# zwpku/colvars-finder

Measured on AMD Instinct MI355X. Metric: MD frames/sec through EigenFunctionTask train step, higher is better.
Workload: dtype f32; 1 GPU; BASELINE config 3: alanine-dipeptide-shaped EigenFunctionTask, generator mode, k=3, 22 atoms, align+position features d_r=66, nets [66,20,20,20,1], diag_coeff, Adam; frames_per_gpu=100000, batch_per_gpu=20000, global_batch=20000, parallelism=dp1 (frames sharded; all-reduce of batch sums + flat gradient)

## Files before the change

### colvars-finder_amd/csrc/ef16_back.hip

```cpp
#include "ef16_common.hpp"

namespace {

struct Back16Args {
  int k;
  int64_t B;
  int64_t n_tiles;
  int64_t T;
  const float* w_lag;
};

template <int H, int NH, bool MULTI, bool GEN>
__global__ __launch_bounds__(256, 4) void ef16_back_kernel(Back16Args args, cvf_mlp_desc mlp, const float* __restrict__ theta,
                                                            const float* __restrict__ packed, const float* __restrict__ w,
                                                            const float* __restrict__ feat, const float* __restrict__ y_tiled,
                                                            const float* __restrict__ q_tiled, const double* __restrict__ coef,
                                                            float* __restrict__ slab, int32_t* __restrict__ step,
                                                            const float* __restrict__ saved) {
  constexpr int RT = Hid<H>::RT, NG = Hid<H>::NG;
  constexpr int RTO = (H + 15) / 16;
  constexpr int CTH = (H + 1 + 15) / 16;
  constexpr int NT = 256, WPB = 4;
  constexpr int kRows = 2 * H + 2 * (H + 1) + 16;
  __shared__ __attribute__((aligned(16))) float IMG[kRows * kPitch];
  __shared__ float PART[4 * (H + 1)];
  extern __shared__ float GI[];
  float* SA1 = IMG;
  float* SA2 = SA1 + H * kPitch;
  float* SB1 = SA2 + H * kPitch;
  float* SB2 = SB1 + (H + 1) * kPitch;
  const int tid = threadIdx.x, lane = tid & 63;
  const int wave = __builtin_amdgcn_readfirstlane(tid >> 6);
  const int col = lane & 15, q = lane >> 4, row16 = col, r0 = 4 * q;
  const int fo = 16 * wave + col;
  const int rowf = 4 * col + q;
  const int net = blockIdx.y, k = args.k, D = mlp.dims[0];
  const int CT1 = (D + 1 + 15) / 16;
  const int c0 = 16 * (CT1 - 1), nfeat = D - c0, ncol = nfeat + 1;
  const bool strip = ncol <= 4;
  const int CTM = strip ? CT1 - 1 : CT1;
  const int gbase = mlp.w_off[net][0];
  const int gspan = mlp.b_off[net][NH] + 1 - gbase;
  float* out = slab + (int64_t)blockIdx.x * mlp.n_params + gbase;

  {
    static_assert((kRows * kPitch) % 4 == 0, "IMG is zeroed in 16-byte pieces");
    float4* img4 = reinterpret_cast<float4*>(IMG);
    for (int i = tid; i < kRows * kPitch / 4; i += NT) img4[i] = float4{0.0f, 0.0f, 0.0f, 0.0f};
  }
  if (MULTI)
    for (int i = tid; i < gspan; i += NT) GI[i] = 0.0f;
  lds_barrier();
  if (tid < 64) SB1[H * kPitch + tid] = 1.0f;

  const PackLayout L = pack_layout(H, NH, D);
  const URows pk = urows(packed + (int64_t)net * L.per_net, L.per_net, lane);
  float wl[RT][4];
  load_hid_const_u<H>(urows(theta + mlp.w_off[net][NH], H, q), wl);
  const double gS1n = coef[net], gEtn = coef[k + k * k + net];
  const double gS1ln = GEN ? 0.0 : coef[2 * k + k * k + net], gS2ln = GEN ? 0.0 : coef[3 * k + k * k + net];
  const float one[1] = {1.0f};

  const __amdgpu_buffer_rsrc_t out_rs = __builtin_amdgcn_make_buffer_rsrc(out, 0, gspan * 4, 0x00020000);
  auto emit_tile = [&](int l, int n_out, int n_in, int rt, int ct, const f32x4& acc) {
    const int wo = mlp.w_off[net][l] - gbase, bo = mlp.b_off[net][l] - gbase;
    const int i = 16 * ct + row16;
    int ob = 16 * rt + r0;
    asm volatile("" : "+v"(ob));
#pragma unroll
    for (int r = 0; r < 4; ++r) {
      const int o = ob + r;
      const bool isw = o < n_out && i < n_in, isb = o < n_out && i == n_in;
      const int idx = isw ? wo + o * n_in + i : bo + (o < n_out ? o : 0);
      const float av = acc[r];
      if (MULTI) {
        if (isw || isb) GI[idx] += av;
      } else {
        __builtin_amdgcn_raw_buffer_store_b32(__builtin_bit_cast(int, av), out_rs, (isw || isb) ? idx * 4 : 0x7ffffff0, 0, 0);
      }
    }
  };
  auto outer2 = [&](const float* A1, const float* B1, const float* A2, const float* B2, int rt, int ct) {
    f32x4 acc = {0.0f, 0.0f, 0.0f, 0.0f};
    acc = outer_half(A1, B1, rt, ct, lane, acc);
    if constexpr (GEN) acc = outer_half(A2, B2, rt, ct, lane, acc);
    return acc;
  };

  auto emit_entry = [&](bool live, int idx, float v) {
    if (MULTI) {
      if (live) GI[idx] += v;
    } else {
      __builtin_amdgcn_raw_buffer_store_b32(__builtin_bit_cast(int, v), out_rs, live ? idx * 4 : 0x7ffffff0, 0, 0);
    }
  };
  auto emit_last = [&]() {
    if (wave == WPB - 1) {
      int i = lane;
      asm volatile("" : "+v"(i));
      const bool live = i <= H;
      const float v = strip_total(PART + (live ? i : H), H + 1);
      emit_entry(live, i < H ? mlp.w_off[net][NH] - gbase + i : mlp.b_off[net][NH] - gbase, v);
    }
  };
  auto emit_strip = [&]() {
    if (strip && 64 * wave < 4 * H) {
      int e = tid;
      asm volatile("" : "+v"(e));
      const int o = e >> 2, c = e & 3;
      const bool live = o < H && c < ncol;
      const float v = strip_total(SB1 + (o < H ? e : 0), 4 * H);
      emit_entry(live, c < nfeat ? mlp.w_off[net][0] - gbase + o * D + c0 + c : mlp.b_off[net][0] - gbase + o, v);
    }
  };

  for (int64_t tile = blockIdx.x; tile < args.n_tiles; tile += gridDim.x) {
    CVF_STAMP(8);
    const bool lagged = !GEN && tile >= args.T;
    const int64_t t0 = lagged ? tile - args.T : tile;
    const int64_t frame = t0 * CVF_TILE + fo;
    const bool valid = frame < args.B;
    const float wraw = w[valid ? frame : args.B - 1];
    float yb[CVF_MAX_NETS];
#pragma unroll
    for (int j = 0; j < CVF_MAX_NETS; ++j) yb[j] = y_tiled[(t0 * k + (j < k ? j : k - 1)) * CVF_TILE + fo];
    float ylag = 0.0f, wlraw = 0.0f;
    if constexpr (!GEN) {
      ylag = y_tiled[((args.T + t0) * k + net) * CVF_TILE + fo];
      wlraw = args.w_lag[valid ? frame : args.B - 1];
    }
    const URows sv = urows(saved + (tile * k + net) * (int64_t)(kHand<NH>() * NG * 256) + wave * 64, kHand<NH>() * NG * 256 - wave * 64, lane);
    Vec<H, 1> h[NH], e[NH > 1 ? NH - 1 : 1], t[NH];
#pragma unroll
    for (int l = 0; l < NH; ++l) {
#pragma unroll
      for (int rt = 0; rt < RT; ++rt) h[l].v[rt][0] = f32x4{0.0f, 0.0f, 0.0f, 0.0f};
#pragma unroll
      for (int g = 0; g < NG; ++g) h[l].v[g >> 2][0][g & 3] = sv.ld((l * NG + g) * 256);
    }
    if constexpr (GEN) {
#pragma unroll
      for (int l = 0; l + 1 < NH; ++l) {
#pragma unroll
        for (int rt = 0; rt < RT; ++rt) e[l].v[rt][0] = f32x4{0.0f, 0.0f, 0.0f, 0.0f};
#pragma unroll
        for (int g = 0; g < NG; ++g) e[l].v[g >> 2][0][g & 3] = sv.ld(((NH + l) * NG + g) * 256);
      }
#pragma unroll
      for (int rt = 0; rt < RT; ++rt) t[0].v[rt][0] = f32x4{0.0f, 0.0f, 0.0f, 0.0f};
#pragma unroll
      for (int g = 0; g < NG; ++g) t[0].v[g >> 2][0][g & 3] = sv.ld(((2 * NH - 1) * NG + g) * 256);
    }
    HFrag<H> ffr[NH > 1 ? NH - 1 : 1];
    if constexpr (GEN) {
#pragma unroll
      for (int l = 1; l < NH; ++l) load_hfrag_u<H>(ffr[l - 1], pk, L.fh(l));
    }
    const float* f_tile = feat + tile * (int64_t)D * CVF_TILE;
    const float* q_tile = GEN ? q_tiled + (tile * k + net) * (int64_t)D * CVF_TILE : nullptr;
    const float wb = valid ? wraw : 0.0f;
    float alpha, gamma = 0.0f;
    float ynet = 0.0f;
#pragma unroll
    for (int j = 0; j < CVF_MAX_NETS; ++j)
      if (j == net) ynet = yb[j];
    if (GEN || !lagged) {
      double a = gS1n;
#pragma unroll
      for (int j = 0; j < CVF_MAX_NETS; ++j)
        if (j < k) a += (j == net ? 2.0 : 1.0) * coef[k + net * k + j] * (double)yb[j];
      alpha = (float)((double)wb * a);
      if constexpr (GEN) gamma = (float)(2.0 * (double)wb * gEtn);
      else alpha = (float)((double)wb * a - 2.0 * (double)wb * gEtn * ((double)ylag - (double)ynet));
    } else {
      const double wlg = valid ? (double)wlraw : 0.0;
      alpha = (float)(wlg * (gS1ln + 2.0 * gS2ln * (double)ylag) + 2.0 * (double)wb * gEtn * ((double)ylag - (double)ynet));
    }
    CVF_STAMP(9);
    if constexpr (GEN) {
#pragma unroll
      for (int rt = 0; rt < RT; ++rt)
#pragma unroll
        for (int r = 0; r < 4; ++r) t[0].v[rt][0][r] *= gamma;
#pragma unroll
      for (int l = 1; l < NH; ++l) {
        Vec<H, 1> td;
        tangent_of<H, 1>(td, h[l - 1], t[l - 1]);
        init_bias<H, 1>(t[l], nullptr, q);
        hidden_mul<H, 1>(t[l], ffr[l - 1], td);
      }
    }
    CVF_STAMP(11);
    {
      const float pick = strip_rows<H>([&](int rt, int r) {
        const float hv = h[NH - 1].v[rt][0][r];
        if constexpr (GEN) return fmaf(alpha, hv, (1.0f - hv * hv) * t[NH - 1].v[rt][0][r]);
        else return alpha * hv;
      }, col);
      const float sa = row_sumf16(alpha);
      if (col < NG && rowf < H) PART[wave * (H + 1) + rowf] = pick;
      if (lane == 0) PART[wave * (H + 1) + H] = sa;
    }
    CVF_STAMP(12);
    Vec<H, 1> hbar;
#pragma unroll
    for (int rt = 0; rt < RT; ++rt)
#pragma unroll
      for (int r = 0; r < 4; ++r) hbar.v[rt][0][r] = alpha * wl[rt][r];
    HFrag<H> tfl;
    float4 bA[4], bB[4];
    float xs[3] = {0.0f, 0.0f, 0.0f}, qs[3] = {0.0f, 0.0f, 0.0f};
    auto request = [&](float4 (&dst)[4], const float* src_tile, int ct) {
      const int i = 16 * ct + row16;
      const float4* p = reinterpret_cast<const float4*>(src_tile + (int64_t)(i < D ? i : D - 1) * CVF_TILE + 4 * q);
#pragma unroll
      for (int j = 0; j < 4; ++j) dst[j] = p[4 * j];
    };
    auto request_step = [&](int l) {
      if (l > 0) {
        load_hfrag_u<H>(tfl, pk, L.th(l));
      } else {
        if (strip) {
#pragma unroll
          for (int c = 0; c < 3; ++c)
            if (c < nfeat) {
              xs[c] = f_tile[(int64_t)(c0 + c) * CVF_TILE + fo];
              if constexpr (GEN) qs[c] = q_tile[(int64_t)(c0 + c) * CVF_TILE + fo];
            }
        }
        request(bA, f_tile, wave);
        if constexpr (GEN) request(bB, q_tile, wave);
      }
    };
    request_step(NH - 1);
#pragma unroll
    for (int l = NH - 1; l >= 0; --l) {
      CVF_STAMP(13 + (NH - 1 - l));
      Vec<H, 1> zbar, dl;
#pragma unroll
      for (int rt = 0; rt < RT; ++rt)
#pragma unroll
        for (int r = 0; r < 4; ++r) {
          const float hv = h[l].v[rt][0][r];
          const float om = 1.0f - hv * hv;
          if constexpr (GEN) {
            const float ev = (l == NH - 1) ? wl[rt][r] : e[l < NH - 1 ? l : 0].v[rt][0][r];
            const float hb = fmaf(-2.0f * hv * t[l].v[rt][0][r], ev, hbar.v[rt][0][r]);
            dl.v[rt][0][r] = ev * om;
            zbar.v[rt][0][r] = om * hb;
          } else {
            zbar.v[rt][0][r] = om * hbar.v[rt][0][r];
          }
        }
      store_image<H, 1, false>(SA1, zbar, one, lane, fo);
      if constexpr (GEN) {
        const float sc[1] = {l == 0 ? gamma : 1.0f};
        store_image<H, 1, true>(SA2, dl, sc, lane, fo);
      }
      if (l > 0) {
        store_image<H, 1, false>(SB1, h[l - 1], one, lane, fo);
        if constexpr (GEN) {
          Vec<H, 1> td;
          tangent_of<H, 1>(td, h[l - 1], t[l - 1]);
          store_image<H, 1, false>(SB2, td, one, lane, fo);
        }
        __syncthreads();
        init_bias<H, 1>(hbar, nullptr, q);
        hidden_mul<H, 1>(hbar, tfl, zbar);
        request_step(l - 1);
        for (int pr = wave; pr < RTO * CTH; pr += WPB) {
          const int rt = pr / CTH, ct = pr - rt * CTH;
          emit_tile(l, H, H, rt, ct, outer2(SA1, SB1, SA2, SB2, rt, ct));
        }
        if (l == NH - 1) emit_last();
        __syncthreads();
      } else {
        if (strip) {
#pragma unroll
          for (int c = 0; c < 4; ++c) {
            if (c < ncol) {
              const float xv = c == nfeat ? 1.0f : xs[c < 3 ? c : 2];
              const float qv = c == nfeat ? 0.0f : gamma * qs[c < 3 ? c : 2];
              const float pick = strip_rows<H>([&](int rt, int r) {
                if constexpr (GEN) return fmaf(zbar.v[rt][0][r], xv, dl.v[rt][0][r] * qv);
                else return zbar.v[rt][0][r] * xv;
              }, col);
              if (col < NG && rowf < H) SB1[(wave * H + rowf) * 4 + c] = pick;
            }
          }
        }
        __syncthreads();
        auto half0 = [&](f32x4 (&acc)[RTO], const float* SA, const float4 (&b)[4], int ct, int rt0, int rstep, bool ones) {
          const int i = 16 * ct + row16;
          const float pad = (ones && i == D) ? 1.0f : 0.0f;
#pragma unroll
          for (int rt = 0; rt < RTO; ++rt) {
            if (rt >= rt0 && (rt - rt0) % rstep == 0) {
              const float4* a1 = reinterpret_cast<const float4*>(SA + (16 * rt + row16) * kPitch + 4 * q);
              float4 av[4];
#pragma unroll
              for (int j = 0; j < 4; ++j) av[j] = a1[4 * j];
#pragma unroll
              for (int j = 0; j < 4; ++j) {
                acc[rt] = mfma4(av[j].x, i < D ? b[j].x : pad, acc[rt]);
                acc[rt] = mfma4(av[j].y, i < D ? b[j].y : pad, acc[rt]);
                acc[rt] = mfma4(av[j].z, i < D ? b[j].z : pad, acc[rt]);
                acc[rt] = mfma4(av[j].w, i < D ? b[j].w : pad, acc[rt]);
              }
            }
          }
        };
        const int extra = (CTM - WPB) * RTO;
        f32x4 acc[RTO];
#pragma unroll
        for (int rt = 0; rt < RTO; ++rt) acc[rt] = f32x4{0.0f, 0.0f, 0.0f, 0.0f};
        if (wave < CTM) {
          half0(acc, SA1, bA, wave, 0, 1, true);
          if (wave < extra) request(bA, f_tile, WPB + wave / RTO);
          if constexpr (GEN) half0(acc, SA2, bB, wave, 0, 1, false);
#pragma unroll
          for (int rt = 0; rt < RTO; ++rt) emit_tile(0, H, D, rt, wave, acc[rt]);
        }
        for (int pr = wave; pr < extra; pr += WPB) {
          const int ct = WPB + pr / RTO, rt = pr % RTO;
          if (pr != wave || wave >= CTM) request(bA, f_tile, ct);
          if constexpr (GEN) request(bB, q_tile, ct);
#pragma unroll
          for (int r_ = 0; r_ < RTO; ++r_) acc[r_] = f32x4{0.0f, 0.0f, 0.0f, 0.0f};
          half0(acc, SA1, bA, ct, rt, RTO, true);
          if constexpr (GEN) half0(acc, SA2, bB, ct, rt, RTO, false);
#pragma unroll
          for (int r_ = 0; r_ < RTO; ++r_)
            if (r_ == rt) emit_tile(0, H, D, r_, ct, acc[r_]);
        }
        emit_strip();
        if (NH == 1) emit_last();
        __syncthreads();
      }
    }
  }
  CVF_STAMP(17);
  if (MULTI) {
    __syncthreads();
    for (int i = tid; i < gspan; i += NT) out[i] = GI[i];
  }
  if (step != nullptr && blockIdx.x == 0 && blockIdx.y == 0 && tid == 0) *step += 1;
  CVF_STAMP(18);
}

}

extern "C" int64_t cvf_ef16_backward_slab_rows(int64_t n_tiles) { return n_tiles < 1024 ? n_tiles : 1024; }

static int ef16_backward_impl(const cvf_ef_cfg* cfg, const cvf_mlp_desc* mlp, const float* theta, const float* packed,
                              int64_t B, const float* w, const float* w_lag, const float* feat_tiled, const float* y_tiled,
                              const float* q_tiled, const double* coef, float* slab, int32_t* step_count, const float* saved,
                              void* stream) {
  const bool transfer = cfg != nullptr && cfg->lag_idx > 0;
  CVF_REQUIRE(cfg && mlp && theta && packed && w && feat_tiled && y_tiled && (transfer ? w_lag != nullptr : q_tiled != nullptr) && coef &&
              slab && saved && B > 0, "cvf_ef16_backward: bad argument");
  CVF_REQUIRE(cfg->k == mlp->n_nets, "cvf_ef16_backward: cfg.k must equal the number of nets");
  int H, NH;
  CVF_REQUIRE(ef16_shape(mlp, &H, &NH), "cvf_ef16_backward: unsupported net shape");
  CVF_REQUIRE(mlp->dims[0] <= 8 * 16 - 1, "cvf_ef16_backward: first layer wider than the column-tile schedule covers");
  const int span = mlp->b_off[0][NH] + 1 - mlp->w_off[0][0];
  int covered = 0;
  for (int n = 0; n < mlp->n_nets; ++n) {
    CVF_REQUIRE(mlp->b_off[n][NH] + 1 - mlp->w_off[n][0] == span, "cvf_ef16_backward: nets are not laid out contiguously");
    for (int l = 0; l <= NH; ++l)
      CVF_REQUIRE(mlp->w_off[n][l] >= mlp->w_off[n][0] && mlp->b_off[n][l] < mlp->w_off[n][0] + span,
                  "cvf_ef16_backward: nets are not laid out contiguously");
    covered += span;
  }
  CVF_REQUIRE(covered == mlp->n_params, "cvf_ef16_backward: flat buffer holds parameters outside the nets");
  Back16Args a;
  a.k = cfg->k;
  a.B = B;
  a.T = cvf_ntiles(B);
  a.n_tiles = transfer ? 2 * a.T : a.T;
  a.w_lag = w_lag;
  const int64_t G = cvf_ef16_backward_slab_rows(a.n_tiles);
  const bool launched = ef16_dispatch(H, NH, [&](auto h_, auto nh_) {
    constexpr int kH = decltype(h_)::value, kNH = decltype(nh_)::value;
    auto go = [&](auto kernel, size_t lds) {
      hipLaunchKernelGGL(kernel, dim3((unsigned)G, cfg->k), dim3(256), lds, (hipStream_t)stream, a, *mlp, theta, packed, w, feat_tiled,
                         y_tiled, q_tiled, coef, slab, step_count, saved);
    };
    const size_t gi = (size_t)span * sizeof(float);
    if (transfer) {
      if (a.n_tiles > G) go(ef16_back_kernel<kH, kNH, true, false>, gi);
      else go(ef16_back_kernel<kH, kNH, false, false>, 0);
    } else {
      if (a.n_tiles > G) go(ef16_back_kernel<kH, kNH, true, true>, gi);
      else go(ef16_back_kernel<kH, kNH, false, true>, 0);
    }
  });
  CVF_REQUIRE(launched, "cvf_ef16_backward: no kernel instance for hidden width %d x %d layers", H, NH);
  return cvf_check_launch("ef16_back_kernel");
}

extern "C" int cvf_ef16_backward(const cvf_ef_cfg* cfg, const cvf_mlp_desc* mlp, const float* theta, const float* packed,
                                 int64_t B, const float* w, const float* feat_tiled, const float* y_tiled, const float* q_tiled,
                                 const double* coef, float* slab, int32_t* step_count, const float* saved, void* stream) {
  CVF_REQUIRE(cfg && cfg->lag_idx == 0, "cvf_ef16_backward: generator mode (transfer-operator mode: cvf_ef16_backward_transfer)");
  return ef16_backward_impl(cfg, mlp, theta, packed, B, w, nullptr, feat_tiled, y_tiled, q_tiled, coef, slab, step_count, saved, stream);
}


extern "C" int cvf_ef16_backward_transfer(const cvf_ef_cfg* cfg, const cvf_mlp_desc* mlp, const float* theta, const float* packed,
                                          int64_t B, const float* w, const float* w_lag, const float* feat_tiled,
                                          const float* y_tiled, const double* coef, float* slab, int32_t* step_count,
                                          const float* saved, void* stream) {
  CVF_REQUIRE(cfg && cfg->lag_idx > 0, "cvf_ef16_backward_transfer: transfer-operator mode (cfg.lag_idx > 0)");
  return ef16_backward_impl(cfg, mlp, theta, packed, B, w, w_lag, feat_tiled, y_tiled, nullptr, coef, slab, step_count, saved, stream);
}
```

### colvars-finder_amd/csrc/ef16_common.hpp

```cpp
#pragma once
#include "cvf_metric.hpp"
#include "ef_frag.hpp"
#include <stdlib.h>
#include <type_traits>


namespace {

constexpr int kU = 16;
constexpr int kImgP = 76;
constexpr int kAuxP = 21;
constexpr int kMaxRows16 = 16384;
template <int NH>
__host__ __device__ constexpr int kHand() { return 2 * NH; }

__device__ __forceinline__ float quad_sumf16(float v) {
  v += dpp_movf<0xB1, 0xf>(v);
  v += dpp_movf<0x4E, 0xf>(v);
  return v;
}
__device__ __forceinline__ double quad_sumd16(double v) {
  v += dpp_movd<0xB1, 0xf>(v);
  v += dpp_movd<0x4E, 0xf>(v);
  return v;
}

__device__ __forceinline__ float row_sumf16(float v) {
  v = quad_sumf16(v);
  v += dpp_movf<0x141, 0xf>(v);
  v += dpp_movf<0x140, 0xf>(v);
  return v;
}
template <int H, class F>
__device__ __forceinline__ float strip_rows(F&& val, int col) {
  float pick = 0.0f;
#pragma unroll
  for (int j = 0; j < Hid<H>::NG; ++j) {
    const float s = row_sumf16(val(j >> 2, j & 3));
    pick = col == j ? s : pick;
  }
  return pick;
}
__device__ __forceinline__ float strip_total(const float* P, int stride) {
  return ((P[0] + P[stride]) + P[2 * stride]) + P[3 * stride];
}

struct Front16Lds {
  int ref, a, aux, w, rs, y, e, feat, g, total;
};
__host__ __device__ inline Front16Lds front16_lds(int nc, int nal, int k) {
  Front16Lds L;
  const int stride = x_tile_stride(nc);
  L.ref = kU * stride;
  L.a = L.ref + 3 * nal;
  L.aux = (L.a + nc + 3) & ~3;
  L.w = L.aux + ((kU * kAuxP + 3) & ~3);
  L.rs = L.w + kU;
  L.y = L.rs + 4;
  L.e = L.y + k * kU;
  L.feat = L.e + k * kU;
  L.g = L.feat + kU * kImgP;
  L.total = L.g + k * kU * kImgP;
  return L;
}

bool ef16_shape(const cvf_mlp_desc* m, int* H, int* NH) {
  if (m->n_layers < 2 || m->n_layers > 4 || m->dims[m->n_layers] != 1) return false;
  *H = m->dims[1];
  *NH = m->n_layers - 1;
  for (int l = 1; l < m->n_layers; ++l)
    if (m->dims[l] != *H) return false;
  for (int l = 0; l < m->n_layers; ++l)
    if (m->act[l] != (l + 1 < m->n_layers ? 1 : 0)) return false;
  return true;
}

template <class F>
bool ef16_dispatch(int H, int NH, F&& f) {
#define EF_CASE(H_, NH_)                                                        \
  if (H == H_ && NH == NH_) {                                                   \
    f(std::integral_constant<int, H_>{}, std::integral_constant<int, NH_>{});   \
    return true;                                                                \
  }
#ifdef CVF_DEV_SHAPES
  EF_CASE(20, 3)
#else
  EF_CASE(8, 1) EF_CASE(8, 2) EF_CASE(8, 3)
  EF_CASE(12, 1) EF_CASE(12, 2) EF_CASE(12, 3)
  EF_CASE(16, 1) EF_CASE(16, 2) EF_CASE(16, 3)
  EF_CASE(20, 1) EF_CASE(20, 2) EF_CASE(20, 3)
  EF_CASE(24, 2) EF_CASE(24, 3)
  EF_CASE(32, 2) EF_CASE(32, 3)
#endif
#undef EF_CASE
  return false;
}

}
```

### colvars-finder_amd/csrc/ef_frag.hpp

```cpp
#pragma once
#include "cvf_common.hpp"
#include "cvf_pack.hpp"

namespace {

typedef float f32x4 __attribute__((ext_vector_type(4)));


constexpr int kPitch = 68;

__device__ __forceinline__ f32x4 mfma4(float a, float b, f32x4 c) {
  return __builtin_amdgcn_mfma_f32_16x16x4f32(a, b, c, 0, 0, 0);
}

template <int H>
struct Hid {
  static constexpr int NG = (H + 3) / 4;
  static constexpr int RT = (NG + 3) / 4;
};

template <int H, int FT>
struct Vec {
  f32x4 v[Hid<H>::RT][FT];
};

template <int H>
__host__ __device__ constexpr int saved_per_vec() { return Hid<H>::NG * 2 * 64 * 2; }
template <int H>
__device__ __forceinline__ void save_vec(float* __restrict__ base, const Vec<H, 4>& X, int lane) {
#pragma unroll
  for (int g = 0; g < Hid<H>::NG; ++g)
#pragma unroll
    for (int w = 0; w < 2; ++w)
      reinterpret_cast<float2*>(base + (g * 2 + w) * 128)[lane] = float2{X.v[g >> 2][2 * w][g & 3], X.v[g >> 2][2 * w + 1][g & 3]};
}
template <int H>
__device__ __forceinline__ void save_vec_half(float* __restrict__ base, const Vec<H, 2>& X, int w, int lane) {
#pragma unroll
  for (int g = 0; g < Hid<H>::NG; ++g)
    reinterpret_cast<float2*>(base + (g * 2 + w) * 128)[lane] = float2{X.v[g >> 2][0][g & 3], X.v[g >> 2][1][g & 3]};
}
template <int H>
__device__ __forceinline__ void load_vec(const float* __restrict__ base, Vec<H, 2>& X, int w, int lane) {
#pragma unroll
  for (int rt = 0; rt < Hid<H>::RT; ++rt)
#pragma unroll
    for (int ft = 0; ft < 2; ++ft) X.v[rt][ft] = f32x4{0.0f, 0.0f, 0.0f, 0.0f};
#pragma unroll
  for (int g = 0; g < Hid<H>::NG; ++g) {
    const float2 t = reinterpret_cast<const float2*>(base + (g * 2 + w) * 128)[lane];
    X.v[g >> 2][0][g & 3] = t.x;
    X.v[g >> 2][1][g & 3] = t.y;
  }
}

template <int H, int FT>
__device__ __forceinline__ void init_bias(Vec<H, FT>& X, const float* __restrict__ b, int q) {
#pragma unroll
  for (int rt = 0; rt < Hid<H>::RT; ++rt) {
    f32x4 bv;
#pragma unroll
    for (int r = 0; r < 4; ++r) {
      const int f = hid_feature(rt, r, q);
      bv[r] = 0.0f;
      if (b != nullptr) {
        const float x = b[f < H ? f : H - 1];
        bv[r] = f < H ? x : 0.0f;
      }
    }
#pragma unroll
    for (int ft = 0; ft < FT; ++ft) X.v[rt][ft] = bv;
  }
}

template <int FT>
__device__ __forceinline__ void load_frames(const float* __restrict__ p, float (&b)[FT]) {
  if constexpr (FT == 4) {
    const float4 v = *reinterpret_cast<const float4*>(p);
    b[0] = v.x; b[1] = v.y; b[2] = v.z; b[3] = v.w;
  } else if constexpr (FT == 2) {
    const float2 v = *reinterpret_cast<const float2*>(p);
    b[0] = v.x; b[1] = v.y;
  } else {
    b[0] = p[0];
  }
}
template <int FT>
__device__ __forceinline__ void store_frames(float* __restrict__ p, const float (&b)[FT]) {
  if constexpr (FT == 4) *reinterpret_cast<float4*>(p) = make_float4(b[0], b[1], b[2], b[3]);
  else if constexpr (FT == 2) *reinterpret_cast<float2*>(p) = make_float2(b[0], b[1]);
  else p[0] = b[0];
}


template <int H>
struct HFrag {
  float a[Hid<H>::NG][Hid<H>::RT];
};
template <int H>
__device__ __forceinline__ void load_hfrag(HFrag<H>& f, const float* __restrict__ pk, int lane) {
#pragma unroll
  for (int s = 0; s < Hid<H>::NG; ++s)
#pragma unroll
    for (int rt = 0; rt < Hid<H>::RT; ++rt) f.a[s][rt] = pk[(unsigned)((s * Hid<H>::RT + rt) * 64) + (unsigned)lane];
}
template <int H, int FT>
__device__ __forceinline__ void hidden_mul(Vec<H, FT>& Y, const HFrag<H>& f, const Vec<H, FT>& X) {
#pragma unroll
  for (int s = 0; s < Hid<H>::NG; ++s)
#pragma unroll
    for (int ft = 0; ft < FT; ++ft)
#pragma unroll
      for (int rt = 0; rt < Hid<H>::RT; ++rt) Y.v[rt][ft] = mfma4(f.a[s][rt], X.v[s >> 2][ft][s & 3], Y.v[rt][ft]);
}
template <int H, int FT>
__device__ __forceinline__ void hidden_apply(Vec<H, FT>& Y, const float* __restrict__ pk, const Vec<H, FT>& X, int lane) {
  HFrag<H> f;
  load_hfrag<H>(f, pk, lane);
  hidden_mul<H, FT>(Y, f, X);
}

template <int H, int FT, int CH>
struct L0Chunk {
  float a[CH][Hid<H>::RT];
  float b[CH][FT];
};
template <int H, int FT, int CH>
__device__ __forceinline__ void load_l0chunk(L0Chunk<H, FT, CH>& c, const float* __restrict__ pk0, int D, int S,
                                             const float* __restrict__ in_lane, int s0, int lane) {
  constexpr int RT = Hid<H>::RT;
  const int q = lane >> 4;
#pragma unroll
  for (int i = 0; i < CH; ++i) {
    const int s = s0 + i;
    const bool live = s < S;
    const int se = live ? s : S - 1;
    const int kf = 4 * se + q;
#pragma unroll
    for (int rt = 0; rt < RT; ++rt) {
#ifdef CVF_EXP_NOW
      const float v = 0.01f * (float)(se + rt);
#else
      const float v = pk0[(se * RT + rt) * 64 + lane];
#endif
      c.a[i][rt] = live ? v : 0.0f;
    }
#ifdef CVF_EXP_NOFEAT
#pragma unroll
    for (int ft = 0; ft < FT; ++ft) c.b[i][ft] = 0.5f + 0.01f * (float)kf;
#else
    load_frames<FT>(in_lane + (int64_t)(kf < D ? kf : 0) * CVF_TILE, c.b[i]);
#endif
  }
}
template <int H, int FT, int CH>
__device__ __forceinline__ void mul_l0chunk(Vec<H, FT>& X, const L0Chunk<H, FT, CH>& c) {
#pragma unroll
  for (int i = 0; i < CH; ++i)
#pragma unroll
    for (int ft = 0; ft < FT; ++ft)
#pragma unroll
      for (int rt = 0; rt < Hid<H>::RT; ++rt) X.v[rt][ft] = mfma4(c.a[i][rt], c.b[i][ft], X.v[rt][ft]);
}
template <int H, int FT, int CH = 6>
__device__ __forceinline__ void layer0_apply(Vec<H, FT>& X, const float* __restrict__ pk0, int D,
                                             const float* __restrict__ in_lane, int lane) {
  const int S = (D + 3) >> 2;
  L0Chunk<H, FT, CH> c0, c1;
  load_l0chunk<H, FT, CH>(c0, pk0, D, S, in_lane, 0, lane);
  for (int s0 = 0; s0 < S; s0 += 2 * CH) {
    load_l0chunk<H, FT, CH>(c1, pk0, D, S, in_lane, s0 + CH, lane);
    mul_l0chunk<H, FT, CH>(X, c0);
    load_l0chunk<H, FT, CH>(c0, pk0, D, S, in_lane, s0 + 2 * CH, lane);
    mul_l0chunk<H, FT, CH>(X, c1);
  }
}

template <int H, int FT, int CH, int NB>
__device__ __forceinline__ void layer0_apply_deep(Vec<H, FT>& X, const float* __restrict__ pk0, int D,
                                                  const float* __restrict__ in_lane, int lane) {
  const int S = (D + 3) >> 2;
  L0Chunk<H, FT, CH> c[NB];
#pragma unroll
  for (int b = 0; b < NB; ++b) load_l0chunk<H, FT, CH>(c[b], pk0, D, S, in_lane, b * CH, lane);
  for (int s0 = 0; s0 < S; s0 += NB * CH) {
#pragma unroll
    for (int b = 0; b < NB; ++b) {
      mul_l0chunk<H, FT, CH>(X, c[b]);
      load_l0chunk<H, FT, CH>(c[b], pk0, D, S, in_lane, s0 + (NB + b) * CH, lane);
    }
  }
}
constexpr int kWideD = 128;

template <int H, int FT, int CH>
__device__ __forceinline__ void layer0_apply_from(Vec<H, FT>& X, const float* __restrict__ pk0, int D,
                                                  const float* __restrict__ in_lane, int lane, L0Chunk<H, FT, CH>& c0) {
  const int S = (D + 3) >> 2;
  L0Chunk<H, FT, CH> c1;
  for (int s0 = 0; s0 < S; s0 += 2 * CH) {
    load_l0chunk<H, FT, CH>(c1, pk0, D, S, in_lane, s0 + CH, lane);
    mul_l0chunk<H, FT, CH>(X, c0);
    load_l0chunk<H, FT, CH>(c0, pk0, D, S, in_lane, s0 + 2 * CH, lane);
    mul_l0chunk<H, FT, CH>(X, c1);
  }
}

template <int H>
struct HConst {
  float c[Hid<H>::RT][4];
};
template <int H>
__device__ __forceinline__ void load_hconst(HConst<H>& o, const float* __restrict__ v, int q) {
#pragma unroll
  for (int rt = 0; rt < Hid<H>::RT; ++rt)
#pragma unroll
    for (int r = 0; r < 4; ++r) {
      const int f = hid_feature(rt, r, q);
      const float x = v[f < H ? f : H - 1];
      o.c[rt][r] = f < H ? x : 0.0f;
    }
}
template <int H, int FT>
__device__ __forceinline__ void set_const(Vec<H, FT>& X, const HConst<H>& b) {
#pragma unroll
  for (int rt = 0; rt < Hid<H>::RT; ++rt)
#pragma unroll
    for (int ft = 0; ft < FT; ++ft)
#pragma unroll
      for (int r = 0; r < 4; ++r) X.v[rt][ft][r] = b.c[rt][r];
}

__device__ __attribute__((noinline)) float ef_act_slow(int act, float z) { return cvf_act(act, z); }
__device__ __attribute__((noinline)) float ef_act_d1_slow(int act, float h) { return cvf_act_d1(act, h); }
__device__ __attribute__((noinline)) float ef_act_d2_slow(int act, float h) { return cvf_act_d2(act, h); }

template <int H, int FT>
__device__ __forceinline__ void tanh_inplace(Vec<H, FT>& X, int act = CVF_ACT_TANH) {
  if (act == CVF_ACT_TANH) {
#pragma unroll
    for (int rt = 0; rt < Hid<H>::RT; ++rt)
#pragma unroll
      for (int ft = 0; ft < FT; ++ft)
#pragma unroll
        for (int r = 0; r < 4; ++r)
          if (4 * rt + r < Hid<H>::NG) X.v[rt][ft][r] = cvf_tanh(X.v[rt][ft][r]);
  } else {
#pragma unroll
    for (int rt = 0; rt < Hid<H>::RT; ++rt)
#pragma unroll
      for (int ft = 0; ft < FT; ++ft)
#pragma unroll
        for (int r = 0; r < 4; ++r)
          if (4 * rt + r < Hid<H>::NG) X.v[rt][ft][r] = ef_act_slow(act, X.v[rt][ft][r]);
  }
}
__device__ __forceinline__ float act_d1(int act, float h) {
  if (act == CVF_ACT_TANH) return 1.0f - h * h;
  return ef_act_d1_slow(act, h);
}

template <int H>
__device__ __forceinline__ void load_hid_const(const float* __restrict__ v, int q, float (&c)[Hid<H>::RT][4]) {
#pragma unroll
  for (int rt = 0; rt < Hid<H>::RT; ++rt)
#pragma unroll
    for (int r = 0; r < 4; ++r) {
      const int f = hid_feature(rt, r, q);
      const float x = v[f < H ? f : H - 1];
      c[rt][r] = f < H ? x : 0.0f;
    }
}

template <int H, int NH, int FT, bool LEAN = false>
__device__ __forceinline__ void chain_forward(const cvf_mlp_desc& mlp, const float* __restrict__ theta,
                                              const float* __restrict__ pk, const PackLayout& L, int net,
                                              const float* __restrict__ in_lane, int lane, Vec<H, FT> (&h)[NH]) {
  const int q = lane >> 4;
  if constexpr (LEAN) {
    init_bias<H, FT>(h[0], theta + mlp.b_off[net][0], q);
    layer0_apply<H, FT, 3>(h[0], pk + L.f0(), mlp.dims[0], in_lane, lane);
    tanh_inplace<H, FT>(h[0], mlp.act[0]);
#pragma unroll
    for (int l = 1; l < NH; ++l) {
      init_bias<H, FT>(h[l], theta + mlp.b_off[net][l], q);
      hidden_apply<H, FT>(h[l], pk + L.fh(l), h[l - 1], lane);
      tanh_inplace<H, FT>(h[l], mlp.act[0]);
    }
    return;
  }
  HConst<H> bias[NH];
#pragma unroll
  for (int l = 0; l < NH; ++l) load_hconst<H>(bias[l], theta + mlp.b_off[net][l], q);
  HFrag<H> hf[NH > 1 ? NH - 1 : 1];
#pragma unroll
  for (int l = 1; l < NH; ++l) load_hfrag<H>(hf[l - 1], pk + L.fh(l), lane);
  CVF_STAMP(1);
  set_const<H, FT>(h[0], bias[0]);
  if (mlp.dims[0] > kWideD) layer0_apply_deep<H, FT, 6, 3>(h[0], pk + L.f0(), mlp.dims[0], in_lane, lane);
  else layer0_apply<H, FT>(h[0], pk + L.f0(), mlp.dims[0], in_lane, lane);
  CVF_STAMP(2);
  tanh_inplace<H, FT>(h[0], mlp.act[0]);
  CVF_STAMP(3);
#pragma unroll
  for (int l = 1; l < NH; ++l) {
    set_const<H, FT>(h[l], bias[l]);
    hidden_mul<H, FT>(h[l], hf[l - 1], h[l - 1]);
    tanh_inplace<H, FT>(h[l], mlp.act[0]);
  }
}

__device__ __forceinline__ float sum_over_q(float v) {
  v += __shfl_xor(v, 16, 64);
  v += __shfl_xor(v, 32, 64);
  return v;
}

struct URows {
  __amdgpu_buffer_rsrc_t r;
  int lane4;
  __device__ __forceinline__ float ld(int float_off) const {
    return __builtin_bit_cast(float, __builtin_amdgcn_raw_buffer_load_b32(r, lane4, float_off * 4, 0));
  }
  __device__ __forceinline__ void st(int float_off, float v) const {
    __builtin_amdgcn_raw_buffer_store_b32(__builtin_bit_cast(int, v), r, lane4, float_off * 4, 0);
  }
};
__device__ __forceinline__ URows urows(const void* base, int n_floats, int lane) {
  return URows{__builtin_amdgcn_make_buffer_rsrc(const_cast<void*>(base), 0, n_floats * 4, 0x00020000), lane * 4};
}
template <int H>
__device__ __forceinline__ void load_hfrag_u(HFrag<H>& f, const URows& u, int off) {
#pragma unroll
  for (int s = 0; s < Hid<H>::NG; ++s)
#pragma unroll
    for (int rt = 0; rt < Hid<H>::RT; ++rt) f.a[s][rt] = u.ld(off + (s * Hid<H>::RT + rt) * 64);
}
template <int H>
__device__ __forceinline__ void load_hid_const_u(const URows& u, float (&c)[Hid<H>::RT][4]) {
#pragma unroll
  for (int rt = 0; rt < Hid<H>::RT; ++rt)
#pragma unroll
    for (int r = 0; r < 4; ++r) c[rt][r] = u.ld(4 * (4 * rt + r));
}

__device__ __forceinline__ f32x4 outer_half(const float* __restrict__ A, const float* __restrict__ B, int rt, int ct,
                                            int lane, f32x4 acc) {
  const int row = lane & 15, kq = lane >> 4;
  const float4* a = reinterpret_cast<const float4*>(A + (16 * rt + row) * kPitch + 4 * kq);
  const float4* b = reinterpret_cast<const float4*>(B + (16 * ct + row) * kPitch + 4 * kq);
  float4 av[4], bv[4];
#pragma unroll
  for (int j = 0; j < 4; ++j) {
    av[j] = a[4 * j];
    bv[j] = b[4 * j];
  }
#pragma unroll
  for (int j = 0; j < 4; ++j) {
    acc = mfma4(av[j].x, bv[j].x, acc);
    acc = mfma4(av[j].y, bv[j].y, acc);
    acc = mfma4(av[j].z, bv[j].z, acc);
    acc = mfma4(av[j].w, bv[j].w, acc);
  }
  return acc;
}
__device__ __forceinline__ f32x4 outer_tile(const float* __restrict__ A1, const float* __restrict__ B1,
                                            const float* __restrict__ A2, const float* __restrict__ B2, int rt, int ct,
                                            bool two, int lane) {
  f32x4 acc = {0.0f, 0.0f, 0.0f, 0.0f};
  acc = outer_half(A1, B1, rt, ct, lane, acc);
  if (two) acc = outer_half(A2, B2, rt, ct, lane, acc);
  return acc;
}

template <int H, int FT, bool SCALE>
__device__ __forceinline__ void store_image(float* S, const Vec<H, FT>& X, const float (&sc)[FT], int lane, int fo) {
  const int q = lane >> 4;
#pragma unroll
  for (int rt = 0; rt < Hid<H>::RT; ++rt)
#pragma unroll
    for (int r = 0; r < 4; ++r) {
      const int f = hid_feature(rt, r, q);
      if (4 * rt + r < Hid<H>::NG && f < H) {
        float v[FT];
#pragma unroll
        for (int ft = 0; ft < FT; ++ft) v[ft] = SCALE ? sc[ft] * X.v[rt][ft][r] : X.v[rt][ft][r];
        float* dst = S + f * kPitch + fo;
        if constexpr (FT == 4) {
          reinterpret_cast<float2*>(dst)[0] = make_float2(v[0], v[1]);
          reinterpret_cast<float2*>(dst)[1] = make_float2(v[2], v[3]);
        } else if constexpr (FT == 2) {
          *reinterpret_cast<float2*>(dst) = make_float2(v[0], v[1]);
        } else {
          dst[0] = v[0];
        }
      }
    }
}

template <int H, int FT>
__device__ __forceinline__ void tangent_of(Vec<H, FT>& td, const Vec<H, FT>& h, const Vec<H, FT>& t, int act = CVF_ACT_TANH) {
  if (act == CVF_ACT_TANH) {
#pragma unroll
    for (int rt = 0; rt < Hid<H>::RT; ++rt)
#pragma unroll
      for (int ft = 0; ft < FT; ++ft)
#pragma unroll
        for (int r = 0; r < 4; ++r) {
          const float hv = h.v[rt][ft][r];
          td.v[rt][ft][r] = (1.0f - hv * hv) * t.v[rt][ft][r];
        }
  } else {
#pragma unroll
    for (int rt = 0; rt < Hid<H>::RT; ++rt)
#pragma unroll
      for (int ft = 0; ft < FT; ++ft)
#pragma unroll
        for (int r = 0; r < 4; ++r) td.v[rt][ft][r] = ef_act_d1_slow(act, h.v[rt][ft][r]) * t.v[rt][ft][r];
  }
}

}
```

Baseline: 328.6 million frames/s.

## Compute ragged hidden-size tail of weight-gradient tiles with 4x4x1 MFMA

When the hidden width leaves a small tail (H mod 16 in 1..4, e.g. H=20), the backward kernel stops computing full 16x16 outer-product tiles for the mostly-empty second row tile. It uses 4x4x1 MFMA blocks instead, then reduces them with permlane swaps and scatters the entries straight into the gradient. Roles rotate across waves by layer parity to balance the work. This cuts wasted MFMA work on padding, at the cost of more complex indexing, extra cross-lane reductions and possible load imbalance between waves.

```diff
diff --git a/colvars-finder_amd/csrc/ef16_back.hip b/colvars-finder_amd/csrc/ef16_back.hip
--- a/colvars-finder_amd/csrc/ef16_back.hip
+++ b/colvars-finder_amd/csrc/ef16_back.hip
@@ -21,6 +21,7 @@
   constexpr int RTO = (H + 15) / 16;
   constexpr int CTH = (H + 1 + 15) / 16;
   constexpr int NT = 256, WPB = 4;
+  constexpr bool TAIL4 = RTO == 2 && H % 16 >= 1 && H % 16 <= 4;
   constexpr int kRows = 2 * H + 2 * (H + 1) + 16;
   __shared__ __attribute__((aligned(16))) float IMG[kRows * kPitch];
   __shared__ float PART[4 * (H + 1)];
@@ -268,9 +269,32 @@
         init_bias<H, 1>(hbar, nullptr, q);
         hidden_mul<H, 1>(hbar, tfl, zbar);
         request_step(l - 1);
-        for (int pr = wave; pr < RTO * CTH; pr += WPB) {
-          const int rt = pr / CTH, ct = pr - rt * CTH;
-          emit_tile(l, H, H, rt, ct, outer2(SA1, SB1, SA2, SB2, rt, ct));
+        if constexpr (TAIL4) {
+          const int role = (wave + 2 * (l & 1)) & 3;
+          if (role == 0) {
+            emit_tile(l, H, H, 0, 0, outer2(SA1, SB1, SA2, SB2, 0, 0));
+          } else {
+            const int g = col >> 2, m = lane & 3;
+            const int wo = mlp.w_off[net][l] - gbase, bo = mlp.b_off[net][l] - gbase;
+            auto job = [&](int arow, int brow, int o, int i, bool live) {
+              f32x4 acc = {0.0f, 0.0f, 0.0f, 0.0f};
+              acc = outer_half44(SA1, arow, SB1, brow, lane, acc);
+              if constexpr (GEN) acc = outer_half44(SA2, arow, SB2, brow, lane, acc);
+              const float v = rows_sum_scatter(acc);
+              asm volatile("" : "+v"(o));
+              live = live && o < H && i <= H;
+              emit_entry(live, i < H ? wo + o * H + i : bo + o, v);
+            };
+            const bool low = role == 1;
+            const int cb = role == 3 ? 20 : 16;
+            job(low ? 16 + m : 4 * g + m, low ? 4 * g + m : cb + m, low ? 16 + q : 4 * g + q, low ? 4 * g + m : cb + m, true);
+            if (low) job(16 + m, 16 + 4 * (g & 1) + m, 16 + q, 16 + 4 * (g & 1) + m, g < 2);
+          }
+        } else {
+          for (int pr = wave; pr < RTO * CTH; pr += WPB) {
+            const int rt = pr / CTH, ct = pr - rt * CTH;
+            emit_tile(l, H, H, rt, ct, outer2(SA1, SB1, SA2, SB2, rt, ct));
+          }
         }
         if (l == NH - 1) emit_last();
         __syncthreads();
@@ -314,12 +338,40 @@
         f32x4 acc[RTO];
 #pragma unroll
         for (int rt = 0; rt < RTO; ++rt) acc[rt] = f32x4{0.0f, 0.0f, 0.0f, 0.0f};
+        auto tail0 = [&](f32x4& tacc, const float* SA, const float4 (&b)[4], int ct, bool ones) {
+          const int i = 16 * ct + row16;
+          const float pad = (ones && i == D) ? 1.0f : 0.0f;
+          const float4* a1 = reinterpret_cast<const float4*>(SA + (16 + (lane & 3)) * kPitch + 4 * q);
+          float4 av[4];
+#pragma unroll
+          for (int j = 0; j < 4; ++j) av[j] = a1[4 * j];
+#pragma unroll
+          for (int j = 0; j < 4; ++j) {
+            tacc = mfma1(av[j].x, i < D ? b[j].x : pad, tacc);
+            tacc = mfma1(av[j].y, i < D ? b[j].y : pad, tacc);
+            tacc = mfma1(av[j].z, i < D ? b[j].z : pad, tacc);
+            tacc = mfma1(av[j].w, i < D ? b[j].w : pad, tacc);
+          }
+        };
         if (wave < CTM) {
-          half0(acc, SA1, bA, wave, 0, 1, true);
+          f32x4 tacc = {0.0f, 0.0f, 0.0f, 0.0f};
+          half0(acc, SA1, bA, wave, 0, TAIL4 ? RTO : 1, true);
+          if constexpr (TAIL4) tail0(tacc, SA1, bA, wave, true);
           if (wave < extra) request(bA, f_tile, WPB + wave / RTO);
-          if constexpr (GEN) half0(acc, SA2, bB, wave, 0, 1, false);
-#pragma unroll
-          for (int rt = 0; rt < RTO; ++rt) emit_tile(0, H, D, rt, wave, acc[rt]);
+          if constexpr (GEN) {
+            half0(acc, SA2, bB, wave, 0, TAIL4 ? RTO : 1, false);
+            if constexpr (TAIL4) tail0(tacc, SA2, bB, wave, false);
+          }
+#pragma unroll
+          for (int rt = 0; rt < (TAIL4 ? 1 : RTO); ++rt) emit_tile(0, H, D, rt, wave, acc[rt]);
+          if constexpr (TAIL4) {
+            const float v = rows_sum_scatter(tacc);
+            int o = 16 + q;
+            asm volatile("" : "+v"(o));
+            const int i = 16 * wave + row16;
+            const bool isw = o < H && i < D, isb = o < H && i == D;
+            emit_entry(isw || isb, isw ? mlp.w_off[net][0] - gbase + o * D + i : mlp.b_off[net][0] - gbase + (o < H ? o : 0), v);
+          }
         }
         for (int pr = wave; pr < extra; pr += WPB) {
           const int ct = WPB + pr / RTO, rt = pr % RTO;
diff --git a/colvars-finder_amd/csrc/ef16_common.hpp b/colvars-finder_amd/csrc/ef16_common.hpp
--- a/colvars-finder_amd/csrc/ef16_common.hpp
+++ b/colvars-finder_amd/csrc/ef16_common.hpp
@@ -43,6 +43,17 @@
 }
 __device__ __forceinline__ float strip_total(const float* P, int stride) {
   return ((P[0] + P[stride]) + P[2 * stride]) + P[3 * stride];
+}
+
+__device__ __forceinline__ float rows_sum_scatter(const f32x4& x) {
+  auto swap_add = [](auto swapped) {
+    const unsigned a = swapped[0], b = swapped[1];
+    return __builtin_bit_cast(float, a) + __builtin_bit_cast(float, b);
+  };
+  const float x0 = x[0], x1 = x[1], x2 = x[2], x3 = x[3];
+  const float s02 = swap_add(__builtin_amdgcn_permlane32_swap(__builtin_bit_cast(unsigned, x0), __builtin_bit_cast(unsigned, x2), false, false));
+  const float s13 = swap_add(__builtin_amdgcn_permlane32_swap(__builtin_bit_cast(unsigned, x1), __builtin_bit_cast(unsigned, x3), false, false));
+  return swap_add(__builtin_amdgcn_permlane16_swap(__builtin_bit_cast(unsigned, s02), __builtin_bit_cast(unsigned, s13), false, false));
 }
 
 struct Front16Lds {
diff --git a/colvars-finder_amd/csrc/ef_frag.hpp b/colvars-finder_amd/csrc/ef_frag.hpp
--- a/colvars-finder_amd/csrc/ef_frag.hpp
+++ b/colvars-finder_amd/csrc/ef_frag.hpp
@@ -11,6 +11,9 @@
 
 __device__ __forceinline__ f32x4 mfma4(float a, float b, f32x4 c) {
   return __builtin_amdgcn_mfma_f32_16x16x4f32(a, b, c, 0, 0, 0);
+}
+__device__ __forceinline__ f32x4 mfma1(float a, float b, f32x4 c) {
+  return __builtin_amdgcn_mfma_f32_4x4x1f32(a, b, c, 0, 0, 0);
 }
 
 template <int H>
@@ -364,6 +367,26 @@
   }
   return acc;
 }
+__device__ __forceinline__ f32x4 outer_half44(const float* __restrict__ A, int arow, const float* __restrict__ B, int brow,
+                                              int lane, f32x4 acc) {
+  const int kq = lane >> 4;
+  const float4* a = reinterpret_cast<const float4*>(A + arow * kPitch + 4 * kq);
+  const float4* b = reinterpret_cast<const float4*>(B + brow * kPitch + 4 * kq);
+  float4 av[4], bv[4];
+#pragma unroll
+  for (int j = 0; j < 4; ++j) {
+    av[j] = a[4 * j];
+    bv[j] = b[4 * j];
+  }
+#pragma unroll
+  for (int j = 0; j < 4; ++j) {
+    acc = mfma1(av[j].x, bv[j].x, acc);
+    acc = mfma1(av[j].y, bv[j].y, acc);
+    acc = mfma1(av[j].z, bv[j].z, acc);
+    acc = mfma1(av[j].w, bv[j].w, acc);
+  }
+  return acc;
+}
 __device__ __forceinline__ f32x4 outer_tile(const float* __restrict__ A1, const float* __restrict__ B1,
                                             const float* __restrict__ A2, const float* __restrict__ B2, int rt, int ct,
                                             bool two, int lane) {
```

After: 340.4 million frames/s (median of 6 runs). 1.04x the previous value.
